# chzhang18/RAG

Hardware: AMD Instinct MI355X
Metric: disparity maps/sec at 384x1248 D=192 (Matching-Net forward) (higher is better)
Workload: dtype f32 (RAGMI_F32X3: level-3/6/12 3x3x3 convolutions with fp32 operands split into power-of-two-scaled FP16 hi+lo halves on the 16-bit matrix cores, hi*hi + hi*lo + lo*hi, fp32 accumulate: fp32-class accuracy, bound in include/rag_amd.h; strict_fp32 holds the RAGMI_F32 number); 1 GPU; BASELINE configs[1]: 1 stereo pair(s)/GPU/step, 384x1248, D=192, f32, all-conv genotype, (left_fea,right_fea)->disp, inputs resident in HBM; global_batch=1, launch=hipGraph, ranks_seen=1

## Files before the change

### include/rag_amd.h

```cpp
#ifndef RAG_AMD_H
#define RAG_AMD_H

#include <stdint.h>

#ifdef __cplusplus
extern "C" {
#endif

#define RAGMI_OK 0
#define RAGMI_EINVAL (-1)
#define RAGMI_EUNSUPPORTED (-2)
#define RAGMI_ELAUNCH (-3)

#define RAGMI_F32 0
#define RAGMI_BF16 1
#define RAGMI_F32X3 2

#define RAGMI_MAX_GROUPS 16

int ragmi_version(void);
const char* ragmi_last_error(void);

int ragmi_costvol_fwd(const void* left_fea, const void* right_fea, void* cost,
                      int B, int C, int d, int h, int w, int dtype, void* stream);

int64_t ragmi_conv3d_k3_packed_elems(int Cout, int Cin);
int ragmi_conv3d_k3_pack(const void* weight, void* packed, int Cout, int Cin, int dtype, void* stream);

int ragmi_conv3d_k3_fwd(const void* x, int64_t x_bstride,
                        const void* packed_weight, const void* scale, const void* shift, int relu,
                        void* y, int64_t y_bstride, const int32_t* y_group_ch,
                        const void* res, int64_t res_bstride, const int32_t* res_group_ch,
                        int B, int Cin, int Cout, int D, int H, int W,
                        int dtype, void* stream);

typedef struct {
  const void* weight;
  const void* scale;
  const void* shift;
  int32_t relu;
  void* y;
  int64_t y_bstride;
  int32_t y_ch0;
  int32_t cout;
} ragmi_tail_t;
int ragmi_down2_tail_supported(int D, int H, int W);

#define RAGMI_CONV_RELU 1
#define RAGMI_CONV_X_G4 2
#define RAGMI_CONV_Y_G4 4
#define RAGMI_TAIL_G4 4
#define RAGMI_TAIL_F32 8
#define RAGMI_TAIL_ROWS 16
#define RAGMI_OUT_F32 0x100
int ragmi_conv3d_k3_g4_caps(int Cin, int Cout, int B, int D, int H, int W, int nset, int ntail, int ndown, int dtype);

#define RAGMI_STORE_QUARTER_ROWS 2
int ragmi_conv3d_k3_quarter_store_supported(int Cin, int Cout, int B, int D, int H, int W, int nset, int ntail, int ndown, int dtype);
int ragmi_quarter_store_rows(int n_in, unsigned char* used);

int ragmi_conv3d_k3_fwd_ex(const void* x, int64_t x_bstride,
                           const void* packed_weight, const void* scale, const void* shift, int relu,
                           void* y, int64_t y_bstride, const int32_t* y_group_ch,
                           const void* res, int64_t res_bstride, const int32_t* res_group_ch,
                           int B, int Cin, int Cout, int D, int H, int W,
                           int store_main, int ntail, const ragmi_tail_t* tails, int dtype, void* stream);
int ragmi_conv3d_k3_dual_fwd_ex(const void* x, int64_t x_bstride,
                                int CinA, const void* packedA, const void* scaleA, const void* shiftA,
                                int CinB, const void* packedB, const void* scaleB, const void* shiftB,
                                int relu, void* y, int64_t y_bstride, const int32_t* y_group_ch,
                                const void* res, int64_t res_bstride, const int32_t* res_group_ch,
                                int B, int Cout, int D, int H, int W,
                                int store_main, int ntail, const ragmi_tail_t* tails, int dtype, void* stream);

int ragmi_conv3d_k3_small_fwd(const void* x, int64_t x_bstride, const void* weight, const void* scale,
                              const void* shift, int relu, void* y, int64_t y_bstride, int y_ch0,
                              const void* res, int64_t res_bstride, int res_ch0,
                              int B, int Cin, int Cout, int D, int H, int W, int dtype, void* stream);

int ragmi_conv3d_k3_small_fwd_ex(const void* x, int64_t x_bstride, const void* weight, const void* scale,
                                 const void* shift, int relu, void* y, int64_t y_bstride, int y_ch0,
                                 const void* res, int64_t res_bstride, int res_ch0,
                                 int B, int Cin, int Cout, int D, int H, int W, int dtype, int y_dtype, void* stream);

int ragmi_conv3d_k3_dual_fwd(const void* x, int64_t x_bstride,
                             int CinA, const void* packedA, const void* scaleA, const void* shiftA,
                             int CinB, const void* packedB, const void* scaleB, const void* shiftB,
                             int relu, void* y, int64_t y_bstride, const int32_t* y_group_ch,
                             const void* res, int64_t res_bstride, const int32_t* res_group_ch,
                             int B, int Cout, int D, int H, int W, int dtype, void* stream);

int ragmi_conv3d_k3_plan(int Cout, int B, int D, int H, int W, int nset, int32_t* log_tx,
                         int32_t* rows_per_lane, int32_t* launch_groups, int32_t max_launches);

int ragmi_conv3d_k1_fwd(const void* x, int64_t x_bstride,
                        const void* weight, const void* scale, const void* shift, int relu,
                        void* y, int64_t y_bstride, int y_ch0,
                        int B, int Cin, int Cout, int64_t DHW,
                        int dtype, void* stream);

int ragmi_conv3d_k1_chain_supported(int Cin, int Cmid, int Cout);
int ragmi_conv3d_k1_chain_fwd(const void* x, int64_t x_bstride, const void* weight1, const void* scale1, const void* shift1, int relu1,
                              int Cmid, const void* weight2, const void* scale2, const void* shift2, int relu2,
// ... 206 lines not shown
```

### rag_amd/csrc/conv3d.hip

```cpp
#include <cstdlib>

#include "conv3d_k3.h"

namespace ragmi {

static int choose_cfg(int B, int D, int H, int W, int Cout = 0) {
#ifdef RAGMI_DIAG
  static const int forced = [] { const char* v = getenv("RAGMI_K3_CFG"); return v ? atoi(v) : -1; }();
  if (forced >= 0) return forced;
#endif
  const int64_t vol = (int64_t)B * D * H * W;
  auto waste = [&](int tx) { return (double)(ceil_div(W, tx) * tx) / W; };
  if (W > 16 && waste(32) <= waste(16) + 1e-9 && vol >= (1 << 20)) return 0;
  if (W > 8 && waste(16) <= waste(8) + 1e-9 && vol >= (1 << 17) && !(Cout >= 20 && vol < (1 << 19))) return 1;
  return 2;
}
int fill_common(K3Args& a, const void* x, int64_t x_bstride, void* y, int64_t y_bstride,
                       const int32_t* y_group_ch, const void* res, int64_t res_bstride, const int32_t* res_group_ch,
                       int B, int Cin, int Cout, int D, int H, int W, int relu) {
  RAGMI_REQUIRE(B > 0 && Cin > 0 && Cout > 0 && D > 0 && H > 0 && W > 0, RAGMI_EINVAL, "conv3d_k3: non-positive size");
  const int ngroups = (Cout + 3) / 4;
  RAGMI_REQUIRE(ngroups <= RAGMI_MAX_GROUPS, RAGMI_EUNSUPPORTED, "conv3d_k3: Cout %d > %d", Cout, 4 * RAGMI_MAX_GROUPS);
  RAGMI_REQUIRE((int64_t)D * H * W < (1ll << 30), RAGMI_EUNSUPPORTED, "conv3d_k3: volume too large (32-bit plane offsets)");
  a.x = x; a.x_bstride = x_bstride;
// ... 49 lines not shown
      ++a.ndown;
      continue;
    }
    const int k = a.ntail;
    RAGMI_REQUIRE(k < 2, RAGMI_EUNSUPPORTED, "conv3d_k3: at most two full-resolution tails");
    RAGMI_REQUIRE(!(tails[t].relu & RAGMI_TAIL_F32), RAGMI_EINVAL, "conv3d_k3: RAGMI_TAIL_F32 is for down-sampling tails");
    const int g4 = (tails[t].relu & RAGMI_TAIL_G4) ? 1 : 0;
    RAGMI_REQUIRE(k == 0 || g4 == a.tail_g4, RAGMI_EUNSUPPORTED, "conv3d_k3: the full-resolution tails of a call share one layout");
    RAGMI_REQUIRE(!g4 || (tails[t].cout == 4 && tails[t].y_ch0 % 4 == 0), RAGMI_EINVAL, "conv3d_k3: a G4 tail has 4 output channels and a group-aligned y_ch0");
    a.tail_g4 = g4;
    a.tail_w[k] = (const float*)tails[t].weight; a.tail_scale[k] = (const float*)tails[t].scale;
    a.tail_shift[k] = (const float*)tails[t].shift; a.tail_y[k] = tails[t].y;
    a.tail_bstride[k] = tails[t].y_bstride; a.tail_ch0[k] = tails[t].y_ch0; a.tail_cout[k] = tails[t].cout;
    a.tail_relu[k] = tails[t].relu & 1;
    ++a.ntail;
  }
  a.store_main = store_main ? 1 : 0;
  return RAGMI_OK;
}

K3Route k3_route(const K3Args& a, int nset, int dtype) {
  if (x2d_eligible(a, nset, dtype)) return K3Route::Split2d;
  if (x3d_eligible(a, nset, dtype)) return K3Route::Box;
  if (!x3_eligible(a, nset, dtype)) return K3Route::Mfma;
#ifndef RAGMI_NO_X3Q
  if (xq_takes(a, nset, dtype)) return K3Route::QuadRing;
#endif
  return K3Route::ZMarch;
}

bool k3_probe(K3Args& a, int Cin, int Cout, int B, int D, int H, int W, int nset, int has_res, int ntail, int ndown) {
  if (Cin <= 0 || Cout <= 0 || B <= 0 || D <= 0 || H <= 0 || W <= 0 || (nset != 1 && nset != 2) || (nset == 2 && Cin % (2 * CK))) return false;
  a = K3Args{};
  a.B = B; a.Cin = Cin; a.Cout = Cout; a.D = D; a.H = H; a.W = W; a.ntail = ntail; a.ndown = ndown;
  a.res = has_res ? (const void*)&a : nullptr;
  for (int t = 0; t < 2; ++t) a.tail_cout[t] = a.down_cout[t] = 4;
  for (int g = 0; g < (Cout + 3) / 4 && g < RAGMI_MAX_GROUPS; ++g) a.y_ch[g] = 4 * g;
  if (nset == 2) a.nchunks[0] = a.nchunks[1] = Cin / (2 * CK);
  else a.nchunks[0] = (Cin + CK - 1) / CK;
  a.store_main = 1;
  return true;
}

static int k3_dispatch(const K3Args& a, int nset, int dtype, hipStream_t s) {
  const char* const who = nset == 2 ? "conv3d_k3_dual" : "conv3d_k3";
  if (a.store_main & RAGMI_STORE_QUARTER_ROWS)
    RAGMI_REQUIRE((a.store_main & 1) && x3_quarter_store_ok(a, nset, dtype), RAGMI_EUNSUPPORTED,
                  "%s: this call does not take RAGMI_STORE_QUARTER_ROWS (ragmi_conv3d_k3_quarter_store_supported)", who);
  const int want = ((a.relu & RAGMI_CONV_X_G4) ? 1 : 0) | (a.tail_g4 ? 2 : 0);
  RAGMI_REQUIRE(!(a.relu & RAGMI_CONV_Y_G4), RAGMI_EUNSUPPORTED, "%s: the main output is channel planes (RAGMI_CONV_Y_G4 not built here)", who);
  RAGMI_REQUIRE((x3_g4_caps(a, nset, dtype) & want) == want, RAGMI_EUNSUPPORTED,
                "%s: this shape / dtype does not take G4 tensors (ragmi_conv3d_k3_g4_caps)", who);
  const K3Route route = k3_route(a, nset, dtype);
  switch (route) {
    case K3Route::Split2d: return x2d_launch(a, nset, dtype, s);
    case K3Route::Box: return x3d_launch(a, nset, dtype, s);
    case K3Route::QuadRing:
    case K3Route::ZMarch: return x3_launch(a, nset, dtype, route, s);
    case K3Route::Mfma: break;
  }
  RAGMI_REQUIRE(a.ndown == 0, RAGMI_EUNSUPPORTED, "%s: down-sampling tails need the z-marching split-operand form (ragmi_conv3d_k3_uses_x3)", who);
  using Launch = int (*)(const K3Args&, int, hipStream_t);
  static const Launch mfma[2][3][2] = {
      {{launch_k3_s1_cfg0_f32, launch_k3_s1_cfg0_bf16}, {launch_k3_s1_cfg1_f32, launch_k3_s1_cfg1_bf16}, {launch_k3_s1_cfg2_f32, launch_k3_s1_cfg2_bf16}},
      {{launch_k3_s2_cfg0_f32, launch_k3_s2_cfg0_bf16}, {launch_k3_s2_cfg1_f32, launch_k3_s2_cfg1_bf16}, {launch_k3_s2_cfg2_f32, launch_k3_s2_cfg2_bf16}}};
  const int cfg = choose_cfg(a.B, a.D, a.H, a.W, a.Cout);
  return mfma[nset - 1][cfg == 0 || cfg == 1 ? cfg : 2][dtype == RAGMI_BF16](a, (a.Cout + 3) / 4, s);
}

}

static int64_t k3_section_elems(int Cout, int Cin) {
  return (int64_t)((Cout + 3) / 4) * ((Cin + ragmi::CK - 1) / ragmi::CK) * ragmi::PACK_PER_GC;
}
extern "C" int64_t ragmi_conv3d_k3_packed_elems(int Cout, int Cin) {
  if (Cout <= 0 || Cin <= 0) return 0;
  return k3_section_elems(Cout, Cin) + ragmi::x3_packed_words(Cout, Cin);
}

extern "C" int ragmi_conv3d_k3_pack(const void* weight, void* packed, int Cout, int Cin, int dtype, void* stream) {
  return ragmi_conv3d_k3_pack_ex(weight, packed, Cout, Cin, 0, 0, dtype, stream);
}

static int pack_sections(const void* weight, void* packed, int Cout, int Cin, int transpose, int planar2d, bool all, void* stream) {
  using namespace ragmi;
  RAGMI_REQUIRE(weight && packed, RAGMI_EINVAL, "conv3d_k3_pack: null pointer");
  RAGMI_REQUIRE(Cout > 0 && Cin > 0, RAGMI_EINVAL, "conv3d_k3_pack: non-positive size");
  RAGMI_REQUIRE(Cout <= 4 * RAGMI_MAX_GROUPS, RAGMI_EUNSUPPORTED, "conv3d_k3_pack: Cout %d > %d", Cout, 4 * RAGMI_MAX_GROUPS);
  const int64_t total = k3_section_elems(Cout, Cin);
  pack_both((const float*)weight, (float*)packed, total, Cout, Cin, transpose ? 1 : 0, planar2d ? 1 : 0, all, static_cast<hipStream_t>(stream));
  return check_launch("conv3d_k3_pack");
}

extern "C" int ragmi_conv3d_k3_pack_ex(const void* weight, void* packed, int Cout, int Cin, int transpose, int planar2d, int dtype,
                                       void* stream) {
  RAGMI_REQUIRE(dtype == RAGMI_F32, RAGMI_EUNSUPPORTED, "conv3d_k3_pack: dtype %d not built", dtype);
  return pack_sections(weight, packed, Cout, Cin, transpose, planar2d, true, stream);
}

extern "C" int ragmi_conv3d_k3_pack_for(const void* weight, void* packed, int Cout, int Cin, int transpose, int planar2d, int for_dtype,
                                        void* stream) {
  RAGMI_REQUIRE(ragmi::conv_dtype_ok(for_dtype), RAGMI_EUNSUPPORTED, "conv3d_k3_pack_for: dtype %d not built", for_dtype);
  return pack_sections(weight, packed, Cout, Cin, transpose, planar2d, for_dtype != RAGMI_F32, stream);
}

extern "C" int ragmi_conv3d_k3_fwd(const void* x, int64_t x_bstride, const void* packed_weight, const void* scale,
// ... 133 lines not shown
```

### rag_amd/csrc/conv3d_x3.hip

```cpp
#include "conv3d_x3_common.h"

namespace ragmi {

#ifdef RAGMI_DIAG
__device__ unsigned long long* x3_stamp_buf = nullptr;
#endif

template <class T, int NCG, int NSET, int TAILS, int XSRC = 0>
__global__ __launch_bounds__(X3_THREADS, (NCG <= 3 ? 4 : 2)) void conv3d_x3_kernel(K3Args a, X3Extra e) {
  constexpr bool BF = std::is_same<T, bf16_t>::value;
  constexpr bool G4X = XSRC == 1, ABX = XSRC == 2;
  constexpr int NCGS = NCG / NSET, NSLS = (NCGS * 27 + 7) / 8, NSL = NSET * NSLS;
  constexpr int NPF = (NCG * X3_PL + X3_THREADS - 1) / X3_THREADS;
  constexpr int RS = x3_row_stride(NCG, NSET), PLS = x3_plane_stride(NCG, NSET), CGS = x3_group_stride(NCG, NSET);
  static_assert(NCG % NSET == 0 && NPF <= 32, "bad instantiation");
  extern __shared__ __attribute__((aligned(16))) uint2 x3_lds[];
  uint2* const lhi = x3_lds;
  uint2* const llo = x3_lds + NCG * CGS;
  uint4* const lw = reinterpret_cast<uint4*>(x3_lds + (BF ? 1 : 2) * NCG * CGS);
  uint4* const ltail = lw + NSL * 2 * 64;
  int2* const loff = reinterpret_cast<int2*>(ltail + 3 * 64);
  float* const par = reinterpret_cast<float*>(loff + 3 * NSL * 4);
  unsigned* const lmaxp = reinterpret_cast<unsigned*>(par + 128);
  float* const ldu = par + 132;
// ... 432 lines not shown
              st4(tbase + ((int64_t)z * HW + (nt & 1) * 16) * 4, u4);
            } else {
              T* pt = tbase + (int64_t)z * HW + (nt & 1) * 16;
#pragma unroll
              for (int r = 0; r < 4; ++r)
                if (r < my_tail_cout) {
                  float u = fmaf(tacc[r], sc4[r], sh4[r]);
                  st(pt + r * DHW, trelu ? fmaxf(u, 0.f) : u);
                }
            }
          }
          if constexpr (TAILS == 2) {
            const int dl = kb - a.ntail;
            if (dl >= 0 && dl < a.ndown) {
              const float4 xt = ldxt[8 * (nt & 1) + (n >> 1)];
              float ux[4];
#pragma unroll
              for (int r = 0; r < 4; ++r) {
                const float p1 = __int_as_float(__builtin_amdgcn_update_dpp(0, __float_as_int(tacc[r]), 0x101, 0xF, 0xF, false));
                ux[r] = lerp2(xt.x, xt.z != 0.f ? p1 : tacc[r], xt.y, p1);
              }
              if (!(n & 1))
                reinterpret_cast<float4*>(ldu)[(((z & 1) * 2 + dl) * X3_TY + (nt >> 1)) * (X3_TX / 2) + 8 * (nt & 1) + (n >> 1)] =
                    make_float4(ux[0], ux[1], ux[2], ux[3]);
            }
          }
        }
      }
      if constexpr (ABX) {
        __builtin_amdgcn_sched_barrier(0);
        prefetch(xb, z + 2);
      }
      X3_STAMP(5);
    }
      if (!again) break;
    }
    if constexpr (TAILS == 2) {
      __syncthreads();
      down_finish(ze - 1, b, y0, x0);
    }
  }
#ifdef RAGMI_DIAG
  if (dg_stamp) {
    X3_STAMP(6);
    unsigned long long* const o = x3_stamp_flush(x3_stamp_buf, dg_sum, dg_steps, dg_t0, dg_r0, wave, lane);
    if (o) o[12] = __builtin_amdgcn_s_getreg((4 << 11) | 20);
  }
#endif
}

constexpr int XD_TY = 8, XD_TX = 16;
constexpr int XD_HY = XD_TY + 2, XD_HX = XD_TX + 2;
constexpr int64_t XD_MIN_VOXELS = 1 << 14;
constexpr int XD_THREADS = 512;

template <class T, int CH8, int NSET, int COGS, bool WS, bool W16 = false>
__global__ __launch_bounds__(W16 ? 1024 : XD_THREADS, W16 ? 1 : (WS ? 4 : 2)) void conv3d_x3d_kernel(K3Args a, X3Extra e) {
  constexpr int THREADS = W16 ? 1024 : XD_THREADS;
  static_assert(!WS || NSET == 2, "per-stage weights only pay with two sets");
  constexpr int XD_TZ = 2, XD_HZ = XD_TZ + 2, XD_PL = XD_HZ * XD_HY * XD_HX, XD_NT = W16 ? 1 : XD_TZ;
  constexpr bool BF = std::is_same<T, bf16_t>::value;
  constexpr int NCG4 = 2 * CH8;
  constexpr int NSLS = (NCG4 * 27 + 7) / 8;
  constexpr int NPF = (NCG4 * XD_PL + THREADS - 1) / THREADS;
  constexpr int REC = CH8 * XD_PL;
  extern __shared__ __attribute__((aligned(16))) uint4 xd_lds[];
  uint4* const lw = xd_lds + (BF ? 1 : 2) * REC;
  float* const par = reinterpret_cast<float*>(lw + (WS ? 1 : NSET) * COGS * NSLS * 2 * 64);
  unsigned* const lmaxp = reinterpret_cast<unsigned*>(par + 2 * NSET * COGS * 16);
  uint2* const lhi2 = reinterpret_cast<uint2*>(xd_lds);
  uint2* const llo2 = reinterpret_cast<uint2*>(xd_lds + REC);
  const int tid = threadIdx.x, wave = tid >> 6, lane = tid & 63, n = lane & 15, kb = lane >> 4;
  const int cog0 = blockIdx.y * COGS, ncog = (a.Cout + 15) >> 4;
  const int HW = a.H * a.W;
  float act_floor = (a.relu & 1) ? 0.f : __builtin_nanf("");
  asm volatile("" : "+v"(act_floor));
  const int64_t DHW = (int64_t)HW * a.D;
  constexpr int NWS = COGS * NSLS * 2 * 64;
  auto wcopy = [&](int set, int region) {
    constexpr int ITER = (NWS + THREADS - 1) / THREADS;
    uint4 wv[ITER];
#pragma unroll
    for (int it = 0; it < ITER; ++it) {
      const int i = min(it * THREADS + tid, NWS - 1);
      const int cl = i / (NSLS * 2 * 64), r = i % (NSLS * 2 * 64);
      const uint4 v = e.wf[set][(int64_t)min(cog0 + cl, ncog - 1) * NSLS * 2 * 64 + r];
      wv[it] = cog0 + cl < ncog ? v : make_uint4(0u, 0u, 0u, 0u);
    }
#pragma unroll
    for (int it = 0; it < ITER; ++it) {
      const int i = it * THREADS + tid;
      if (i < NWS) lw[region * NWS + i] = wv[it];
    }
  };
#ifdef RAGMI_DIAG
  const bool diag_nowcopy = (a.relu & 0x800) != 0;
#else
  constexpr bool diag_nowcopy = false;
#endif
  float pf[NPF][4];
  unsigned valid = 0;
  const T* const x = static_cast<const T*>(a.x);
  int offs[NPF];
  auto locate = [&](int z0, int y0, int x0) {
    valid = 0;
#pragma unroll
    for (int p = 0; p < NPF; ++p) {
      const int el = p * THREADS + tid, cg4 = el / XD_PL, r = el % XD_PL;
      const int xx = r % XD_HX, yy = (r / XD_HX) % XD_HY, zz = r / (XD_HX * XD_HY);
      const int gz = z0 - 1 + zz, gy = y0 - 1 + yy, gx = x0 - 1 + xx;
      const bool ok = cg4 < NCG4 && (unsigned)gz < (unsigned)a.D && (unsigned)gy < (unsigned)a.H && (unsigned)gx < (unsigned)a.W;
      valid |= (ok ? 1u : 0u) << p;
      offs[p] = (int)(min(cg4, NCG4 - 1) * 4 * DHW) + min(max(gz, 0), a.D - 1) * HW + min(max(gy, 0), a.H - 1) * a.W + min(max(gx, 0), a.W - 1);
    }
  };
  auto prefetch = [&](const T* xb, int set) {
    const T* xs = xb + (int64_t)set * (8 * CH8) * DHW;
#pragma unroll
    for (int p = 0; p < NPF; ++p)
#pragma unroll
      for (int c = 0; c < 4; ++c) pf[p][c] = ld(xs + c * DHW + offs[p]);
  };
  auto commit = [&](float mul) {
#pragma unroll
    for (int p = 0; p < NPF; ++p) {
      const int el = p * THREADS + tid;
      if (el >= NCG4 * XD_PL) continue;
      const int cg4 = el / XD_PL, r = el % XD_PL;
      const bool ok = (valid >> p) & 1u;
      unsigned l01, l23, h01, h23;
      if constexpr (BF) {
        h01 = x3_split2(ok ? pf[p][0] : 0.f, ok ? pf[p][1] : 0.f, l01); h23 = x3_split2(ok ? pf[p][2] : 0.f, ok ? pf[p][3] : 0.f, l23);
      } else {
        h01 = x3_split2h(ok ? pf[p][0] : 0.f, ok ? pf[p][1] : 0.f, mul, l01); h23 = x3_split2h(ok ? pf[p][2] : 0.f, ok ? pf[p][3] : 0.f, mul, l23);
      }
      const int d = ((cg4 >> 1) * XD_PL + r) * 2 + (cg4 & 1);
      lhi2[d] = make_uint2(h01, h23);
      if constexpr (!BF) llo2[d] = make_uint2(l01, l23);
    }
  };
  const int tz = W16 ? wave >> 3 : wave >> 2, ty0 = W16 ? (wave & 7) : (wave & 3) * 2;
  const int vb0 = (((CH8 == 2 ? (kb & 1) : 0) * XD_PL) + (tz * XD_HY + ty0) * XD_HX + n) * (int)sizeof(uint4);
  int vsl[NSLS];
#pragma unroll
  for (int sl = 0; sl < NSLS; ++sl) {
    const int tap = min(CH8 == 2 ? 2 * sl + (kb >> 1) : 4 * sl + kb, 26);
    vsl[sl] = vb0 + ((tap / 9 * XD_HY + (tap / 3) % 3) * XD_HX + tap % 3) * (int)sizeof(uint4);
  }
  const char* const lbytes = reinterpret_cast<const char*>(xd_lds);
  constexpr int LO_BYTES = REC * (int)sizeof(uint4);
  const int ngroups = (a.Cout + 3) >> 2;
  int my_ych[COGS];
#pragma unroll
  for (int cl = 0; cl < COGS; ++cl) {
    const int g = (cog0 + cl) * 4 + kb;
    my_ych[cl] = g < ngroups ? a.y_ch[g < RAGMI_MAX_GROUPS ? g : 0] : 0;
  }
  auto decode = [&](int work, int& b, int& z0, int& y0, int& x0) {
    int t = work;
    x0 = (t % a.tiles_x) * XD_TX; t /= a.tiles_x;
    y0 = (t % a.tiles_y) * XD_TY; t /= a.tiles_y;
    z0 = (t % a.tiles_z) * XD_TZ; b = t / a.tiles_z;
  };
  const int chunk = (e.nwork + 7) / 8;
  auto work_of = [&](int j) { return (j >> 3) < chunk ? (j & 7) * chunk + (j >> 3) : e.nwork; };
  int j = blockIdx.x;
  while (j < chunk * 8 && work_of(j) >= e.nwork) j += gridDim.x;
  int b = 0, z0 = 0, y0 = 0, x0 = 0, stage = 0;
  if (j < chunk * 8) {
    decode(work_of(j), b, z0, y0, x0);
    locate(z0, y0, x0);
    prefetch(x + b * a.x_bstride, 0);
  }
  if constexpr (!WS) {
    if (!diag_nowcopy)
#pragma unroll
    for (int set = 0; set < NSET; ++set) wcopy(set, set);
  }
#pragma unroll
  for (int set = 0; set < NSET; ++set) {
    const float* const psc = a.scale[set];
    const float* const psh = a.shift[set];
    if (tid < COGS * 16) {
      const int co = cog0 * 16 + tid, cc = min(co, a.Cout - 1);
      const float vsc = psc ? psc[cc] : 1.f, vsh = psh ? psh[cc] : 0.f;
      float sc = co < a.Cout ? vsc : 1.f;
      if constexpr (!BF) { const float wm = e.wmul[set][cc]; sc *= (co < a.Cout ? wm : 1.f); }
      par[set * COGS * 16 + tid] = sc;
      par[NSET * COGS * 16 + set * COGS * 16 + tid] = co < a.Cout ? vsh : 0.f;
    }
  }
  if (tid < 3) lmaxp[tid] = 0u;
  __syncthreads();
#ifdef RAGMI_DIAG
  const bool diag_nostore = (a.relu & 0x100) != 0, diag_nomfma = (a.relu & 0x200) != 0, diag_nostage = (a.relu & 0x400) != 0;
#else
  constexpr bool diag_nostore = false, diag_nomfma = false, diag_nostage = false;
#endif
  while (j < chunk * 8) {
    int jn = j + gridDim.x;
    while (jn < chunk * 8 && work_of(jn) >= e.nwork) jn += gridDim.x;
    int bn = b, zn = z0, yn = y0, xn = x0;
    if (jn < chunk * 8) decode(work_of(jn), bn, zn, yn, xn);
    f32x4 acc[NSET][COGS][XD_NT];
    float inv_mul[NSET];
#pragma unroll
    for (int st = 0; st < NSET; ++st) {
      inv_mul[st] = 1.f;
#pragma unroll
      for (int cl = 0; cl < COGS; ++cl)
#pragma unroll
        for (int i = 0; i < XD_NT; ++i) acc[st][cl][i] = f32x4{0.f, 0.f, 0.f, 0.f};
    }
    static_for<NSET>([&](auto st_) {
      constexpr int st = decltype(st_)::value;
      float mul = 1.f;
      __builtin_amdgcn_sched_barrier(0);
      if constexpr (!BF) {
        float m = 0.f;
#pragma unroll
        for (int p = 0; p < NPF; ++p) {
          const float mp = x3_scalable_max4(pf[p][0], pf[p][1], pf[p][2], pf[p][3]);
          m = fmaxf(m, ((valid >> p) & 1u) ? mp : 0.f);
        }
        m = x3_wave_max(m);
        if (lane == 0) atomicMax(lmaxp + stage % 3, __float_as_uint(m));
      }
      __syncthreads();
      if constexpr (!BF) {
        mul = x3_pow2_scale(__uint_as_float(lmaxp[stage % 3]), 16384.f);
        inv_mul[st] = 1.f / mul;
      }
      if (!diag_nostage) commit(mul);
      if constexpr (WS) wcopy(st, 0);
      __syncthreads();
      if constexpr (!BF) {
        if (tid == 0) lmaxp[(stage + 2) % 3] = 0u;
        ++stage;
      }
      if (!diag_nostage) {
        if constexpr (st + 1 < NSET) prefetch(x + b * a.x_bstride, st + 1);
        else { locate(zn, yn, xn); prefetch(x + bn * a.x_bstride, 0); }
      }
      __builtin_amdgcn_sched_barrier(0);
      if (!diag_nomfma)
#pragma unroll
      for (int sl = 0; sl < NSLS; ++sl) {
        constexpr int ROWB = XD_HX * (int)sizeof(uint4);
        uint4 bh[XD_NT], bl[XD_NT];
#pragma unroll
        for (int i = 0; i < XD_NT; ++i) {
          const int d = (i & 1) * ROWB + (i >> 1) * 2 * XD_HY * ROWB;
          bh[i] = *reinterpret_cast<const uint4*>(lbytes + vsl[sl] + d);
          if constexpr (!BF) bl[i] = *reinterpret_cast<const uint4*>(lbytes + vsl[sl] + d + LO_BYTES);
        }
#pragma unroll
        for (int cl = 0; cl < COGS; ++cl) {
          constexpr int wr = WS ? 0 : st;
          const uint4 ah = lw[(((wr * COGS + cl) * NSLS + sl) * 2 + 0) * 64 + lane];
          const uint4 al = lw[(((wr * COGS + cl) * NSLS + sl) * 2 + 1) * 64 + lane];
#pragma unroll
          for (int i = 0; i < XD_NT; ++i) acc[st][cl][i] = x3_mma<BF>(ah, bh[i], acc[st][cl][i]);
          if constexpr (!BF)
#pragma unroll
          for (int i = 0; i < XD_NT; ++i) acc[st][cl][i] = x3_mma<BF>(ah, bl[i], acc[st][cl][i]);
#pragma unroll
          for (int i = 0; i < XD_NT; ++i) acc[st][cl][i] = x3_mma<BF>(al, bh[i], acc[st][cl][i]);
        }
      }
    });
#pragma unroll
    for (int cl = 0; cl < COGS; ++cl) {
      const int g = (cog0 + cl) * 4 + kb;
#pragma unroll
      for (int i = 0; i < XD_NT; ++i) {
        const int gz = z0 + tz + 2 * (i >> 1), gy = y0 + ty0 + (i & 1), gx = x0 + n;
        const bool inside = gz < a.D && gy < a.H && gx < a.W;
        float v[4];
#pragma unroll
        for (int r = 0; r < 4; ++r) {
          float sum = 0.f;
#pragma unroll
          for (int st = 0; st < NSET; ++st) {
            const float u = fmaxf(fmaf(acc[st][cl][i][r], par[(st * COGS + cl) * 16 + 4 * kb + r] * inv_mul[st], par[NSET * COGS * 16 + (st * COGS + cl) * 16 + 4 * kb + r]), act_floor);
            sum = st == 0 ? u : sum + u;
          }
          v[r] = sum;
        }
        if (inside && g < ngroups && !(diag_nostore && v[0] != 12345.f)) {
          T* py = static_cast<T*>(a.y) + b * a.y_bstride + (int64_t)my_ych[cl] * DHW + ((int64_t)gz * HW + gy * a.W + gx);
#pragma unroll
          for (int r = 0; r < 4; ++r) st(py + r * DHW, v[r]);
        }
      }
    }
    j = jn; b = bn; z0 = zn; y0 = yn; x0 = xn;
  }
}

bool x3d_eligible(const K3Args& a, int nset, int dtype) {
  if ((dtype != RAGMI_F32X3 && dtype != RAGMI_BF16) || a.res != nullptr || a.ntail > 0 || a.ndown > 0 || !a.store_main) return false;
  const int nc = a.nchunks[0];
  if ((nc != 2 && nc != 4) || (nset == 2 && a.nchunks[1] != nc) || a.Cin != nset * nc * 4 || a.Cout % 4 != 0) return false;
  if (a.D < 2 || a.W < 8 || (int64_t)a.D * a.H * a.W < XD_MIN_VOXELS || (int64_t)a.Cin * a.D * a.H * a.W >= (1ll << 31)) return false;
  return true;
}

template <class T, int CH8, int NSET, int COGS, bool WS, bool W16 = false>
static int x3d_launch_one(K3Args a, X3Extra e, hipStream_t st) {
  constexpr int THREADS = W16 ? 1024 : XD_THREADS;
  constexpr int PL = 4 * XD_HY * XD_HX;
  constexpr size_t lds = (size_t)(std::is_same<T, bf16_t>::value ? 1 : 2) * CH8 * PL * sizeof(uint4) +
                         (size_t)(WS ? 1 : NSET) * COGS * ((2 * CH8 * 27 + 7) / 8) * 2 * 64 * sizeof(uint4) + (size_t)(2 * NSET * COGS * 16 + 4) * sizeof(float);
  static_assert(lds <= 160 * 1024, "deep-level tile does not fit the LDS");
  a.tiles_x = (int)ceil_div(a.W, XD_TX); a.tiles_y = (int)ceil_div(a.H, XD_TY); a.tiles_z = (int)ceil_div(a.D, 2);
  const int64_t nwork = (int64_t)a.tiles_x * a.tiles_y * a.tiles_z * a.B;
  RAGMI_REQUIRE(nwork < (1ll << 28), RAGMI_EUNSUPPORTED, "conv3d_x3d: too many tiles");
  e.nwork = (int)nwork;
  static LaunchState state;
  const int slots = state.slots((const void*)conv3d_x3d_kernel<T, CH8, NSET, COGS, WS, W16>, THREADS, lds, 160 * 1024);
  if (slots <= 0) return fail(RAGMI_ELAUNCH, "conv3d_x3d: cannot raise the dynamic LDS limit");
  const int ny = (int)ceil_div((a.Cout + 15) / 16, COGS);
  int64_t gx = std::max<int64_t>(1, std::min<int64_t>(e.nwork, slots / ny));
  if (gx >= 8) gx -= gx % 8;
  hipLaunchKernelGGL((conv3d_x3d_kernel<T, CH8, NSET, COGS, WS, W16>), dim3((unsigned)gx, (unsigned)ny), dim3(THREADS), lds, st, a, e);
  return check_launch("conv3d_x3d");
}

int x3d_launch(K3Args a, int nset, int dtype, hipStream_t st) {
#ifdef RAGMI_DIAG
  static const int diag_xd = [] { const char* v = getenv("RAGMI_XD_DIAG"); return v ? atoi(v) : 0; }();
  a.relu |= diag_xd << 8;
#endif
  X3Extra e{};
  x3_weight_sections(e, a, nset, dtype);
  const bool bf = dtype == RAGMI_BF16;
  const int ch8 = a.nchunks[0] / 2;
#define RAGMI_XD(CH8_, NSET_, COGS_, WS_) (bf ? x3d_launch_one<bf16_t, CH8_, NSET_, COGS_, WS_>(a, e, st) : x3d_launch_one<float, CH8_, NSET_, COGS_, WS_>(a, e, st))
#ifndef RAGMI_XD_COGS1
  if (ch8 == 1 && nset == 2 && a.Cout > 16) return RAGMI_XD(1, 2, 2, false);
#endif
  if (ch8 == 1) return nset == 2 ? RAGMI_XD(1, 2, 1, false) : RAGMI_XD(1, 1, 1, false);
#ifndef RAGMI_XD_NOW16
  if (nset == 2) return bf ? x3d_launch_one<bf16_t, 2, 2, 1, false, true>(a, e, st) : x3d_launch_one<float, 2, 2, 1, false, true>(a, e, st);
#endif
  return nset == 2 ? RAGMI_XD(2, 2, 1, false) : RAGMI_XD(2, 1, 1, false);
#undef RAGMI_XD
}

int64_t x3_packed_words(int Cout, int Cin) {
  return 2 * x3_frag_words(Cout, Cin) + (int64_t)((Cout + 15) / 16) * 16;
}

__global__ void pack_both_kernel(const float* __restrict__ w, float* __restrict__ packed, int64_t total_k3, int nb_k3, int nb_x3, int Cout, int Cin,
                                 int nchunks, int nsls, int ncog, int transpose, int planar, int poison) {
  if ((int)blockIdx.x < nb_k3) {
    const int64_t idx = (int64_t)blockIdx.x * 256 + threadIdx.x;
    if (idx < total_k3) packed[idx] = k3_pack_value(w, Cout, Cin, nchunks, idx, transpose, planar);
    if (poison && blockIdx.x == 0) {
      const int64_t fw = (int64_t)ncog * nsls * 2 * 64 * 4;
      unsigned* const sec = reinterpret_cast<unsigned*>(packed + total_k3);
      for (int c = 0; c < ncog; ++c)
        for (int i = threadIdx.x; i < 256; i += 256) {
          sec[(int64_t)c * nsls * 2 * 64 * 4 + i] = 0x7fc07fc0u;
          sec[fw + (int64_t)c * nsls * 2 * 64 * 4 + i] = 0x7e007e00u;
        }
      for (int i = threadIdx.x; i < ncog * 16; i += 256) sec[2 * fw + i] = 0x7fc00000u;
    }
  } else {
    const int half = ((int)blockIdx.x - nb_k3) >= nb_x3 ? 1 : 0;
    __shared__ unsigned rowmax[64];
    if (half) x3_row_max(w, rowmax, Cout, Cin, transpose, planar, (int)threadIdx.x, 256);
    const int64_t fw = (int64_t)ncog * nsls * 2 * 64 * 4;
    x3_pack_one(w, reinterpret_cast<uint4*>(packed + total_k3 + half * fw), packed + total_k3 + 2 * fw, rowmax, Cout, Cin, nsls, ncog, transpose, planar,
                half, ((int)blockIdx.x - nb_k3 - half * nb_x3) * 256 + threadIdx.x);
  }
}
int pack_both(const float* w, float* packed, int64_t total_k3, int Cout, int Cin, int transpose, int planar, bool all, hipStream_t s) {
  const int ncgs = (Cin + 3) / 4, nsls = (ncgs * 27 + 7) / 8, ncog = (Cout + 15) / 16;
  const int nb_k3 = (int)ceil_div(total_k3, 256), nb_x3 = (int)ceil_div((int64_t)ncog * nsls * 64, 256);
  hipLaunchKernelGGL(pack_both_kernel, dim3((unsigned)(nb_k3 + (all ? 2 * nb_x3 : 0))), dim3(256), 0, s, w, packed, total_k3, nb_k3, nb_x3, Cout, Cin,
                     (Cin + CK - 1) / CK, nsls, ncog, transpose, planar, all ? 0 : 1);
  return RAGMI_OK;
}

bool x3_eligible(const K3Args& a, int nset, int dtype) {
  if ((dtype != RAGMI_F32X3 && dtype != RAGMI_BF16) || a.res != nullptr) return false;
  if (a.Cin % 4 != 0 || a.Cout % 4 != 0) return false;
  const int ncg = a.nchunks[0] + (nset == 2 ? a.nchunks[1] : 0);
  if (nset == 2 && (a.nchunks[0] != a.nchunks[1] || a.nchunks[0] > 2)) return false;
  if (nset == 1 && ncg > 6) return false;
  if ((int64_t)a.D * a.H * a.W < X3_MIN_VOXELS || a.W < 32 || a.D < 8) return false;
  if ((a.ntail > 0 || a.ndown > 0) && a.Cout > 16) return false;
  if ((int64_t)a.Cin * a.D * a.H * a.W >= (1ll << 31)) return false;
  return true;
// ... 154 lines not shown
```

### rag_amd/ops.py

```python
from __future__ import annotations

import ctypes
import os
from typing import List, Optional, Sequence

import torch

from ._lib import K1RSpec, TailSpec, check, load_library

F32, BF16, F32X3 = 0, 1, 2
_DT = {torch.float32: F32, torch.bfloat16: BF16}

_CONV_PRECISIONS = ("f16x3", "fp32")
_PRECISION_ALIASES = {"bf16x3": "f16x3", "split": "f16x3"}
_conv_precision = "fp32" if os.environ.get("RAGMI_X3", "1").strip() == "0" else "f16x3"


def set_conv_precision(precision: str) -> str:
    global _conv_precision
    precision = _PRECISION_ALIASES.get(precision, precision)
    if precision not in _CONV_PRECISIONS:
        raise ValueError(f"conv precision must be one of {_CONV_PRECISIONS}, got {precision!r}")
    old, _conv_precision = _conv_precision, precision
    return old


def get_conv_precision() -> str:
    return _conv_precision


class conv_precision:

    def __init__(self, precision: str):
        self.precision = precision

    def __enter__(self):
        self.old = set_conv_precision(self.precision)
        return self

    def __exit__(self, *exc):
        set_conv_precision(self.old)
        return False


def _conv_dt(dt: int) -> int:
    return F32X3 if (dt == F32 and _conv_precision == "f16x3") else dt


def _stream() -> int:
    return torch.cuda.current_stream().cuda_stream


def _need_gpu(*ts: torch.Tensor) -> None:
    for t in ts:
        if t is None:
            continue
        if not t.is_cuda:
# ... 330 lines not shown
        raise ValueError("conv3d_k3: destination channels exceed the output buffer")
    ntail, tarr = _tail_array(tails)
    check(load_library().ragmi_conv3d_k3_fwd_ex(
        x.data_ptr(), xb, packed.data_ptr(),
        scale.data_ptr() if scale is not None else None, shift.data_ptr() if shift is not None else None, int(relu) | (CONV_X_G4 if x_g4 else 0),
        out.data_ptr(), yb, _i32_array(out_group_ch),
        res.data_ptr() if res is not None else None, rb, _i32_array(res_group_ch),
        B, Cin, cout, D, H, W, int(store_main), ntail, tarr, _conv_dt(dt), _stream()), "conv3d_k3")
    return out


def conv3d_k3_small(x: torch.Tensor, weight: torch.Tensor, scale, shift, relu: bool, out: torch.Tensor, out_ch0: int = 0,
                    res: Optional[torch.Tensor] = None, res_ch0: int = 0) -> torch.Tensor:
    _need_gpu(weight, scale, shift)
    dt = _act(x, res)
    ydt = _act(out)
    if ydt != dt and not (dt == BF16 and ydt == F32):
        raise RuntimeError("conv3d_k3_small: out must have x's dtype (or be float32 when x is bfloat16)")
    B, Cin, D, H, W = x.shape
    cout = weight.shape[0]
    w = weight.detach().contiguous()
    if out_ch0 + cout > out.shape[1] or tuple(out.shape[2:]) != (D, H, W):
        raise ValueError("conv3d_k3_small: output buffer too small / wrong spatial size")
    ptr = lambda t: t.data_ptr() if t is not None else None
    check(load_library().ragmi_conv3d_k3_small_fwd_ex(
        x.data_ptr(), _planes(x), w.data_ptr(), ptr(scale), ptr(shift), int(relu), out.data_ptr(), _planes(out), out_ch0,
        ptr(res), _planes(res) if res is not None else 0, res_ch0, B, Cin, cout, D, H, W, dt, ydt, _stream()), "conv3d_k3_small")
    return out


def conv3d_k3_dual(x: torch.Tensor, cin_a: int, packed_a: torch.Tensor, scale_a, shift_a,
                   packed_b: torch.Tensor, scale_b, shift_b, cout: int, relu: bool, out: torch.Tensor,
                   out_group_ch: Optional[Sequence[int]] = None, res: Optional[torch.Tensor] = None,
                   res_group_ch: Optional[Sequence[int]] = None, tails: Optional[Sequence[Tail]] = None,
                   store_main: bool = True, x_g4: bool = False, quarter: bool = False) -> torch.Tensor:
    if quarter and not store_main:
        raise ValueError("conv3d_k3_dual: quarter=True qualifies a main store")
    if x_g4 and not x.is_contiguous():
        raise ValueError("conv3d_k3_dual: a G4 input is a contiguous buffer")
    _need_gpu(packed_a, packed_b, scale_a, shift_a, scale_b, shift_b)
    dt = _act_with_tails(x, out, res, tails)
    B, Cx, D, H, W = x.shape
    ng = packed_groups(cout)
    if out_group_ch is not None and len(out_group_ch) != ng:
        raise ValueError("conv3d_k3_dual: out_group_ch needs one entry per group of 4 output channels")
    if res is not None and res_group_ch is None:
        res_group_ch = out_group_ch
    if tuple(out.shape[2:]) != (D, H, W) or out.shape[0] != B or not 0 < cin_a < Cx:
        raise ValueError("conv3d_k3_dual: bad shapes")
    ptr = lambda t: t.data_ptr() if t is not None else None
    ntail, tarr = _tail_array(tails)
    check(load_library().ragmi_conv3d_k3_dual_fwd_ex(
        x.data_ptr(), _planes(x), cin_a, packed_a.data_ptr(), ptr(scale_a), ptr(shift_a),
        Cx - cin_a, packed_b.data_ptr(), ptr(scale_b), ptr(shift_b), int(relu) | (CONV_X_G4 if x_g4 else 0),
        out.data_ptr(), _planes(out), _i32_array(out_group_ch),
        ptr(res), _planes(res) if res is not None else 0, _i32_array(res_group_ch),
        B, cout, D, H, W, int(store_main) | (STORE_QUARTER_ROWS if quarter else 0), ntail, tarr, _conv_dt(dt), _stream()), "conv3d_k3_dual")
    return out


def conv3d_k1(x: torch.Tensor, weight2d: torch.Tensor, scale: Optional[torch.Tensor], shift: Optional[torch.Tensor],
              relu: bool, out: torch.Tensor, out_ch0: int = 0, transposed: bool = False) -> torch.Tensor:
    _need_gpu(weight2d, scale, shift)
    dt = _act(x, out)
    B, Cin = x.shape[:2]
    Cout = weight2d.shape[1 if transposed else 0]
    if not weight2d.is_contiguous() or weight2d.shape[0 if transposed else 1] != Cin:
        raise ValueError("conv3d_k1: weight must be contiguous [Cout, Cin] (or [Cin, Cout] with transposed=True)")
    dhw = 1
    for s in x.shape[2:]:
        dhw *= s
    if out_ch0 + Cout > out.shape[1] or tuple(out.shape[2:]) != tuple(x.shape[2:]):
        raise ValueError("conv3d_k1: output buffer too small / wrong spatial size")
    check(load_library().ragmi_conv3d_k1_fwd_ex(
        x.data_ptr(), _planes(x), weight2d.data_ptr(), int(transposed),
        scale.data_ptr() if scale is not None else None, shift.data_ptr() if shift is not None else None, int(relu),
        out.data_ptr(), _planes(out), out_ch0, B, Cin, Cout, dhw, dt, _stream()), "conv3d_k1")
    return out


_CHAIN_K1 = [os.environ.get("RAGMI_CHAIN_K1", "1") != "0"]


def set_chain_k1(enabled: bool) -> None:
    _CHAIN_K1[0] = bool(enabled)


def chain_k1_enabled() -> bool:
    return _CHAIN_K1[0]


def conv3d_k1_chain_supported(cin: int, cmid: int, cout: int) -> bool:
    return bool(load_library().ragmi_conv3d_k1_chain_supported(int(cin), int(cmid), int(cout)))


def conv3d_k1_chain(x: torch.Tensor, w1: torch.Tensor, scale1, shift1, relu1: bool, w2: torch.Tensor, scale2, shift2, relu2: bool,
                    out: torch.Tensor, out_ch0: int = 0) -> torch.Tensor:
    _need_gpu(w1, scale1, shift1, w2, scale2, shift2)
    dt = _act(x, out)
    B, Cin = x.shape[:2]
    Cmid, Cout = w1.shape[0], w2.shape[0]
    if not (w1.is_contiguous() and w2.is_contiguous()) or w1.shape[1] != Cin or w2.shape[1] != Cmid:
        raise ValueError("conv3d_k1_chain: weights must be contiguous [Cmid, Cin] and [Cout, Cmid]")
    dhw = 1
    for sdim in x.shape[2:]:
        dhw *= sdim
    if out_ch0 + Cout > out.shape[1] or tuple(out.shape[2:]) != tuple(x.shape[2:]):
        raise ValueError("conv3d_k1_chain: output buffer too small / wrong spatial size")
    p = lambda t: t.data_ptr() if t is not None else None
    check(load_library().ragmi_conv3d_k1_chain_fwd(x.data_ptr(), _planes(x), w1.data_ptr(), p(scale1), p(shift1), int(relu1), Cmid,
                                                   w2.data_ptr(), p(scale2), p(shift2), int(relu2), out.data_ptr(), _planes(out), out_ch0,
                                                   B, Cin, Cout, dhw, dt, _stream()), "conv3d_k1_chain")
    return out


def conv3d_k1_resample(x: torch.Tensor, size: Sequence[int], align_corners: bool, weight2d: torch.Tensor,
                       scale: Optional[torch.Tensor], shift: Optional[torch.Tensor], relu: bool, out: torch.Tensor,
                       out_ch0: int = 0) -> torch.Tensor:
    _need_gpu(weight2d, scale, shift)
    if x.dtype == torch.bfloat16 and out.dtype == torch.float32:
        dt = _act(x) | OUT_F32
        _act(out)
    else:
        dt = _act(x, out)
    B, Cin, Di, Hi, Wi = x.shape
    Do, Ho, Wo = [int(v) for v in size]
    Cout = weight2d.shape[0]
    if out_ch0 + Cout > out.shape[1] or tuple(out.shape[2:]) != (Do, Ho, Wo):
        raise ValueError("conv3d_k1_resample: output buffer too small / wrong spatial size")
    check(load_library().ragmi_conv3d_k1_resample_fwd(
        x.data_ptr(), _planes(x), Di, Hi, Wi, weight2d.data_ptr(),
# ... 524 lines not shown
```

Measured before the change: 1108 disparity maps/s.

## Add three-output-block weight-streaming variant of the deep-level dual conv box kernel

Adds a COGS=3, weight-streaming 1024-thread instantiation of the deep-level box kernel for f32x3 dual convs with Cout 33-48 and 4+4 input chunks. The variant is used when all tiles fit in one wave of resident blocks. Next-stage weights are loaded into registers before the MFMA loop and written to LDS after it, so the weight copy overlaps compute. Tap offsets and output-channel indices are computed on the fly instead of held in per-thread tables to save registers. A plan query flag and Python knobs (env RAGMI_XD_THREE_BLOCKS) are also added. The cost is lower per-block weight reuse and more register pressure from the in-flight weights.

```diff
diff --git a/include/rag_amd.h b/include/rag_amd.h
--- a/include/rag_amd.h
+++ b/include/rag_amd.h
@@ -49,6 +49,9 @@
 #define RAGMI_CONV_RELU 1
 #define RAGMI_CONV_X_G4 2
 #define RAGMI_CONV_Y_G4 4
+#define RAGMI_CONV_XD_BLOCKS1 8
+#define RAGMI_CONV_XD_PLAN 16
+#define RAGMI_CONV_XD_BLOCKS3 32
 #define RAGMI_TAIL_G4 4
 #define RAGMI_TAIL_F32 8
 #define RAGMI_TAIL_ROWS 16
diff --git a/rag_amd/csrc/conv3d.hip b/rag_amd/csrc/conv3d.hip
--- a/rag_amd/csrc/conv3d.hip
+++ b/rag_amd/csrc/conv3d.hip
@@ -125,6 +125,7 @@
   RAGMI_REQUIRE((x3_g4_caps(a, nset, dtype) & want) == want, RAGMI_EUNSUPPORTED,
                 "%s: this shape / dtype does not take G4 tensors (ragmi_conv3d_k3_g4_caps)", who);
   const K3Route route = k3_route(a, nset, dtype);
+  if ((a.relu & RAGMI_CONV_XD_PLAN) && route != K3Route::Box) return 0;
   switch (route) {
     case K3Route::Split2d: return x2d_launch(a, nset, dtype, s);
     case K3Route::Box: return x3d_launch(a, nset, dtype, s);
diff --git a/rag_amd/csrc/conv3d_x3.hip b/rag_amd/csrc/conv3d_x3.hip
--- a/rag_amd/csrc/conv3d_x3.hip
+++ b/rag_amd/csrc/conv3d_x3.hip
@@ -508,6 +508,7 @@
 constexpr int XD_TY = 8, XD_TX = 16;
 constexpr int XD_HY = XD_TY + 2, XD_HX = XD_TX + 2;
 constexpr int64_t XD_MIN_VOXELS = 1 << 14;
+constexpr int xd_tap_bytes(int tap) { return ((tap / 9 * XD_HY + (tap / 3) % 3) * XD_HX + tap % 3) * (int)sizeof(uint4); }
 constexpr int XD_THREADS = 512;
 
 template <class T, int CH8, int NSET, int COGS, bool WS, bool W16 = false>
@@ -532,6 +533,10 @@
   float act_floor = (a.relu & 1) ? 0.f : __builtin_nanf("");
   asm volatile("" : "+v"(act_floor));
   const int64_t DHW = (int64_t)HW * a.D;
+  auto fresh = [](int v) {
+    if constexpr (WS) asm volatile("" : "+v"(v));
+    return v;
+  };
   constexpr int NWS = COGS * NSLS * 2 * 64;
   auto wcopy = [&](int set, int region) {
     constexpr int ITER = (NWS + THREADS - 1) / THREADS;
@@ -547,6 +552,25 @@
     for (int it = 0; it < ITER; ++it) {
       const int i = it * THREADS + tid;
       if (i < NWS) lw[region * NWS + i] = wv[it];
+    }
+  };
+  constexpr int WITER = WS ? (NWS + THREADS - 1) / THREADS : 1;
+  uint4 wv[WITER];
+  const unsigned wbase = (unsigned)cog0 * (NSLS * 2 * 64), wend = (unsigned)ncog * (NSLS * 2 * 64);
+  auto wload = [&](int set) {
+    const char* const wf = reinterpret_cast<const char*>(e.wf[set]);
+#pragma unroll
+    for (int it = 0; it < WITER; ++it) {
+      unsigned off = min(wbase + (unsigned)(it * THREADS + tid), wend - 1u) * (unsigned)sizeof(uint4);
+      asm volatile("" : "+v"(off));
+      wv[it] = *reinterpret_cast<const uint4*>(wf + off);
+    }
+  };
+  auto wstore = [&]() {
+#pragma unroll
+    for (int it = 0; it < WITER; ++it) {
+      const int i = it * THREADS + fresh(tid);
+      if (i < NWS) lw[i] = wbase + (unsigned)i < wend ? wv[it] : make_uint4(0u, 0u, 0u, 0u);
     }
   };
 #ifdef RAGMI_DIAG
@@ -562,7 +586,7 @@
     valid = 0;
 #pragma unroll
     for (int p = 0; p < NPF; ++p) {
-      const int el = p * THREADS + tid, cg4 = el / XD_PL, r = el % XD_PL;
+      const int el = p * THREADS + fresh(tid), cg4 = el / XD_PL, r = el % XD_PL;
       const int xx = r % XD_HX, yy = (r / XD_HX) % XD_HY, zz = r / (XD_HX * XD_HY);
       const int gz = z0 - 1 + zz, gy = y0 - 1 + yy, gx = x0 - 1 + xx;
       const bool ok = cg4 < NCG4 && (unsigned)gz < (unsigned)a.D && (unsigned)gy < (unsigned)a.H && (unsigned)gx < (unsigned)a.W;
@@ -601,8 +625,10 @@
 #pragma unroll
   for (int sl = 0; sl < NSLS; ++sl) {
     const int tap = min(CH8 == 2 ? 2 * sl + (kb >> 1) : 4 * sl + kb, 26);
-    vsl[sl] = vb0 + ((tap / 9 * XD_HY + (tap / 3) % 3) * XD_HX + tap % 3) * (int)sizeof(uint4);
-  }
+    vsl[sl] = vb0 + xd_tap_bytes(tap);
+  }
+  static_assert(!WS || CH8 == 2, "the table-free K loop is written for two taps per slice");
+  const int odd_tap = -(kb >> 1);
   const char* const lbytes = reinterpret_cast<const char*>(xd_lds);
   constexpr int LO_BYTES = REC * (int)sizeof(uint4);
   const int ngroups = (a.Cout + 3) >> 2;
@@ -611,6 +637,11 @@
   for (int cl = 0; cl < COGS; ++cl) {
     const int g = (cog0 + cl) * 4 + kb;
     my_ych[cl] = g < ngroups ? a.y_ch[g < RAGMI_MAX_GROUPS ? g : 0] : 0;
+  }
+  int* const ychl = reinterpret_cast<int*>(lmaxp + 4);
+  if constexpr (WS) {
+    const int g = cog0 * 4 + tid;
+    if (tid < COGS * 4) ychl[tid] = g < ngroups ? a.y_ch[g < RAGMI_MAX_GROUPS ? g : 0] : 0;
   }
   auto decode = [&](int work, int& b, int& z0, int& y0, int& x0) {
     int t = work;
@@ -632,7 +663,10 @@
     if (!diag_nowcopy)
 #pragma unroll
     for (int set = 0; set < NSET; ++set) wcopy(set, set);
-  }
+  } else {
+    if (!diag_nowcopy) { wload(0); wstore(); }
+  }
+  bool wpend = false;
 #pragma unroll
   for (int set = 0; set < NSET; ++set) {
     const float* const psc = a.scale[set];
@@ -688,7 +722,9 @@
         inv_mul[st] = 1.f / mul;
       }
       if (!diag_nostage) commit(mul);
-      if constexpr (WS) wcopy(st, 0);
+      if constexpr (WS) {
+        if (wpend) wstore();
+      }
       __syncthreads();
       if constexpr (!BF) {
         if (tid == 0) lmaxp[(stage + 2) % 3] = 0u;
@@ -698,17 +734,25 @@
         if constexpr (st + 1 < NSET) prefetch(x + b * a.x_bstride, st + 1);
         else { locate(zn, yn, xn); prefetch(x + bn * a.x_bstride, 0); }
       }
+      if constexpr (WS) {
+        wpend = !diag_nowcopy && (st + 1 < NSET || jn < chunk * 8);
+        if (wpend) wload((st + 1) % NSET);
+      }
       __builtin_amdgcn_sched_barrier(0);
+      const int vbs = fresh(vb0);
       if (!diag_nomfma)
 #pragma unroll
       for (int sl = 0; sl < NSLS; ++sl) {
         constexpr int ROWB = XD_HX * (int)sizeof(uint4);
+        int vs;
+        if constexpr (WS) vs = vbs + xd_tap_bytes(2 * sl) + (odd_tap & (xd_tap_bytes(min(2 * sl + 1, 26)) - xd_tap_bytes(2 * sl)));
+        else vs = vsl[sl];
         uint4 bh[XD_NT], bl[XD_NT];
 #pragma unroll
         for (int i = 0; i < XD_NT; ++i) {
           const int d = (i & 1) * ROWB + (i >> 1) * 2 * XD_HY * ROWB;
-          bh[i] = *reinterpret_cast<const uint4*>(lbytes + vsl[sl] + d);
-          if constexpr (!BF) bl[i] = *reinterpret_cast<const uint4*>(lbytes + vsl[sl] + d + LO_BYTES);
+          bh[i] = *reinterpret_cast<const uint4*>(lbytes + vs + d);
+          if constexpr (!BF) bl[i] = *reinterpret_cast<const uint4*>(lbytes + vs + d + LO_BYTES);
         }
 #pragma unroll
         for (int cl = 0; cl < COGS; ++cl) {
@@ -727,7 +771,15 @@
     });
 #pragma unroll
     for (int cl = 0; cl < COGS; ++cl) {
-      const int g = (cog0 + cl) * 4 + kb;
+      if constexpr (WS) __builtin_amdgcn_sched_barrier(0);
+      const int g = (cog0 + cl) * 4 + kb, pk = fresh(4 * kb);
+      int ych = my_ych[cl];
+      float floor_v = act_floor;
+      if constexpr (WS) {
+        ych = ychl[cl * 4 + (pk >> 2)];
+        floor_v = (a.relu & 1) ? 0.f : __builtin_nanf("");
+        asm volatile("" : "+v"(floor_v));
+      }
 #pragma unroll
       for (int i = 0; i < XD_NT; ++i) {
         const int gz = z0 + tz + 2 * (i >> 1), gy = y0 + ty0 + (i & 1), gx = x0 + n;
@@ -738,13 +790,13 @@
           float sum = 0.f;
 #pragma unroll
           for (int st = 0; st < NSET; ++st) {
-            const float u = fmaxf(fmaf(acc[st][cl][i][r], par[(st * COGS + cl) * 16 + 4 * kb + r] * inv_mul[st], par[NSET * COGS * 16 + (st * COGS + cl) * 16 + 4 * kb + r]), act_floor);
+            const float u = fmaxf(fmaf(acc[st][cl][i][r], par[(st * COGS + cl) * 16 + pk + r] * inv_mul[st], par[NSET * COGS * 16 + (st * COGS + cl) * 16 + pk + r]), floor_v);
             sum = st == 0 ? u : sum + u;
           }
           v[r] = sum;
         }
         if (inside && g < ngroups && !(diag_nostore && v[0] != 12345.f)) {
-          T* py = static_cast<T*>(a.y) + b * a.y_bstride + (int64_t)my_ych[cl] * DHW + ((int64_t)gz * HW + gy * a.W + gx);
+          T* py = static_cast<T*>(a.y) + b * a.y_bstride + (int64_t)ych * DHW + ((int64_t)gz * HW + gy * a.W + gx);
 #pragma unroll
           for (int r = 0; r < 4; ++r) st(py + r * DHW, v[r]);
         }
@@ -762,20 +814,32 @@
   return true;
 }
 
+static bool x3d_three_blocks(const K3Args& a, int nset, int dtype) {
+  return dtype == RAGMI_F32X3 && nset == 2 && a.nchunks[0] == 4 && a.nchunks[1] == 4 && a.Cout > 32 && a.Cout <= 48 && a.Cout % 4 == 0 &&
+         !(a.relu & RAGMI_CONV_XD_BLOCKS1);
+}
+
+constexpr int XD_DECLINED = 1 << 30;
+constexpr int XD_PLAN_SLOTS = 256;
+
 template <class T, int CH8, int NSET, int COGS, bool WS, bool W16 = false>
-static int x3d_launch_one(K3Args a, X3Extra e, hipStream_t st) {
+static int x3d_launch_one(K3Args a, X3Extra e, hipStream_t st, bool one_box_only = false) {
   constexpr int THREADS = W16 ? 1024 : XD_THREADS;
   constexpr int PL = 4 * XD_HY * XD_HX;
   constexpr size_t lds = (size_t)(std::is_same<T, bf16_t>::value ? 1 : 2) * CH8 * PL * sizeof(uint4) +
-                         (size_t)(WS ? 1 : NSET) * COGS * ((2 * CH8 * 27 + 7) / 8) * 2 * 64 * sizeof(uint4) + (size_t)(2 * NSET * COGS * 16 + 4) * sizeof(float);
+                         (size_t)(WS ? 1 : NSET) * COGS * ((2 * CH8 * 27 + 7) / 8) * 2 * 64 * sizeof(uint4) + (size_t)(2 * NSET * COGS * 16 + 4 + (WS ? COGS * 4 : 0)) * sizeof(float);
   static_assert(lds <= 160 * 1024, "deep-level tile does not fit the LDS");
   a.tiles_x = (int)ceil_div(a.W, XD_TX); a.tiles_y = (int)ceil_div(a.H, XD_TY); a.tiles_z = (int)ceil_div(a.D, 2);
   const int64_t nwork = (int64_t)a.tiles_x * a.tiles_y * a.tiles_z * a.B;
   RAGMI_REQUIRE(nwork < (1ll << 28), RAGMI_EUNSUPPORTED, "conv3d_x3d: too many tiles");
   e.nwork = (int)nwork;
+  const bool plan = (a.relu & RAGMI_CONV_XD_PLAN) != 0;
   static LaunchState state;
-  const int slots = state.slots((const void*)conv3d_x3d_kernel<T, CH8, NSET, COGS, WS, W16>, THREADS, lds, 160 * 1024);
+  int slots = (!plan || one_box_only) ? state.slots((const void*)conv3d_x3d_kernel<T, CH8, NSET, COGS, WS, W16>, THREADS, lds, 160 * 1024) : 0;
+  if (plan && slots <= 0) slots = XD_PLAN_SLOTS;
   if (slots <= 0) return fail(RAGMI_ELAUNCH, "conv3d_x3d: cannot raise the dynamic LDS limit");
+  if (one_box_only && nwork > slots) return XD_DECLINED;
+  if (plan) return (COGS << 20) | (int)lds;
   const int ny = (int)ceil_div((a.Cout + 15) / 16, COGS);
   int64_t gx = std::max<int64_t>(1, std::min<int64_t>(e.nwork, slots / ny));
   if (gx >= 8) gx -= gx % 8;
@@ -797,6 +861,12 @@
   if (ch8 == 1 && nset == 2 && a.Cout > 16) return RAGMI_XD(1, 2, 2, false);
 #endif
   if (ch8 == 1) return nset == 2 ? RAGMI_XD(1, 2, 1, false) : RAGMI_XD(1, 1, 1, false);
+#ifndef RAGMI_XD_NOCOGS3
+  if (x3d_three_blocks(a, nset, dtype)) {
+    const int rc = x3d_launch_one<float, 2, 2, 3, true, true>(a, e, st, !(a.relu & RAGMI_CONV_XD_BLOCKS3));
+    if (rc != XD_DECLINED) return rc;
+  }
+#endif
 #ifndef RAGMI_XD_NOW16
   if (nset == 2) return bf ? x3d_launch_one<bf16_t, 2, 2, 1, false, true>(a, e, st) : x3d_launch_one<float, 2, 2, 1, false, true>(a, e, st);
 #endif
diff --git a/rag_amd/ops.py b/rag_amd/ops.py
--- a/rag_amd/ops.py
+++ b/rag_amd/ops.py
@@ -2,7 +2,7 @@
 
 import ctypes
 import os
-from typing import List, Optional, Sequence
+from typing import List, Optional, Sequence, Tuple
 
 import torch
 
@@ -439,7 +439,8 @@
     ntail, tarr = _tail_array(tails)
     check(load_library().ragmi_conv3d_k3_dual_fwd_ex(
         x.data_ptr(), _planes(x), cin_a, packed_a.data_ptr(), ptr(scale_a), ptr(shift_a),
-        Cx - cin_a, packed_b.data_ptr(), ptr(scale_b), ptr(shift_b), int(relu) | (CONV_X_G4 if x_g4 else 0),
+        Cx - cin_a, packed_b.data_ptr(), ptr(scale_b), ptr(shift_b),
+        int(relu) | (CONV_X_G4 if x_g4 else 0) | _xd_flags(),
         out.data_ptr(), _planes(out), _i32_array(out_group_ch),
         ptr(res), _planes(res) if res is not None else 0, _i32_array(res_group_ch),
         B, cout, D, H, W, int(store_main) | (STORE_QUARTER_ROWS if quarter else 0), ntail, tarr, _conv_dt(dt), _stream()), "conv3d_k3_dual")
@@ -464,6 +465,33 @@
         scale.data_ptr() if scale is not None else None, shift.data_ptr() if shift is not None else None, int(relu),
         out.data_ptr(), _planes(out), out_ch0, B, Cin, Cout, dhw, dt, _stream()), "conv3d_k1")
     return out
+
+
+CONV_XD_BLOCKS1, CONV_XD_PLAN, CONV_XD_BLOCKS3 = 8, 16, 32
+_XD_THREE_BLOCKS = [int(os.environ.get("RAGMI_XD_THREE_BLOCKS", "1"))]
+
+
+def set_xd_three_blocks(enabled: bool, any_batch: bool = False) -> None:
+    _XD_THREE_BLOCKS[0] = (2 if any_batch else 1) if enabled else 0
+
+
+def xd_three_blocks_enabled() -> bool:
+    return _XD_THREE_BLOCKS[0] != 0
+
+
+def _xd_flags() -> int:
+    return (CONV_XD_BLOCKS1, 0, CONV_XD_BLOCKS3)[_XD_THREE_BLOCKS[0]]
+
+
+def conv3d_k3_dual_box_plan(cin_a: int, cin_b: int, cout: int, B: int, D: int, H: int, W: int,
+                            dtype: torch.dtype = torch.float32) -> Optional[Tuple[int, int]]:
+    fake = ctypes.c_void_p(0x1000)
+    flags = CONV_XD_PLAN | _xd_flags()
+    rc = load_library().ragmi_conv3d_k3_dual_fwd_ex(fake, 0, cin_a, fake, None, None, cin_b, fake, None, None, flags, fake, 0, None,
+                                                    None, 0, None, B, cout, D, H, W, 1, 0, None, _conv_dt(_DT[dtype]), None)
+    if rc < 0:
+        check(rc, "conv3d_k3_dual_box_plan")
+    return (rc >> 20, rc & 0xFFFFF) if rc > 0 else None
 
 
 _CHAIN_K1 = [os.environ.get("RAGMI_CHAIN_K1", "1") != "0"]
```

After: 1104 disparity maps/s. Within noise of the previous version (-0.4%).
